# sandflow/ffmpeg-ht

Measured on AMD Instinct MI355X. Metric: Mpixels/s HTJ2K decode (4K lossless 5/3) at 1/2/4/8 GPU; IDWT HBM GB/s vs peak, higher is better.
Workload: dtype int32 (int16 storage); 1 GPU; configs[1]: 3840x2160 RGB 8-bit lossless 5/3 + RCT, 64x64 codeblocks, 5 levels, single tile, HT cleanup pass only; 128 frames per step per GPU as 2 concurrent jobs (HIP streams; the frame pipeline keeps that many in flight), device-resident input (codeblock bytes + descriptors) and output (rgb24); jobs=2, distinct_frames=4, block_errors=0

## Files before the change

ffmpeg-ht_amd/csrc/ht_kernels.hpp:

```cpp
#pragma once
#include <hip/hip_runtime.h>
#include <stdint.h>
#include "j2k_plan.h"

namespace htj2k {

struct HtLds {
    uint32_t off_ms, ms_words;
    uint32_t off_vlc, vlc_words;
    uint32_t off_suf, suf_bytes;
    uint32_t off_qinfo, max_qw;
    uint32_t off_E;
    uint32_t off_bm, bm_words;
    uint32_t total;
};

#define HT_ERR_INVALID 1
#define HT_REF_STRIDE 64
#define HT_MEL_SYMS  1344
#define HT_MEL_WORDS (HT_MEL_SYMS / 32 + 2)
#define HT_UVLC_ENTRIES (5 * 64)
#define HT_VSTAGE_PITCH 17
#define HT_VSTAGE_BYTES (64 * HT_VSTAGE_PITCH * 4)

// ... 269 lines not shown
        pv[jx] = pi * 8 < Pcup ? Dq[pi] : make_uint2(0u, 0u);
    }
#pragma unroll
    for (int jx = 0; jx < 4; jx++)
        if (512u * jx < Pcup) ht_unstuff_magsgn_step8(pv[jx], 64 * jx, Pcup, ms, lane, base, carry);
    for (uint32_t p0 = 256; p0 * 8 < Pcup; p0 += 64) {
        const uint32_t pi = p0 + lane;
        ht_unstuff_magsgn_step8(pi * 8 < Pcup ? Dq[pi] : make_uint2(0u, 0u), p0, Pcup, ms, lane, base, carry);
    }
    return base;
}

template <int TRANSFORM, bool REFINE, bool C16 = false>
__device__ __forceinline__ int ht_magsgn_rows_narrow(const ht_sym_t *__restrict__ qglob, const uint32_t *ms,
                                                     uint32_t *__restrict__ dst, int lane, int w, int h,
                                                     int stride, int pLSB, int maxbp, int M_b, float fscale, int i_step,
                                                     uint32_t last_wi, uint32_t *__restrict__ sink,
                                                     const uint64_t *__restrict__ rb, int z_blk)
{
    const int qw = (w + 1) >> 1, qh = (h + 1) >> 1;
    const int col = lane;
    const bool act = col < 2 * qw;
    const bool st_ok = col < w;
    const int q = col >> 1, sh = (col & 1) * 2;
    const int dshift = 31 - M_b;
    const uint32_t half = 1u << ((pLSB - 1) & 31);
    const bool direct53 = pLSB >= dshift && pLSB >= 1 && pLSB <= 30;
    const uint32_t keep53 = (uint32_t)(31 - pLSB) & 31u, up53 = (uint32_t)(pLSB - dshift) & 31u, hb53 = (half & 0x7FFFFFFFu) >> (dshift & 31);
    uint32_t ms_pos = 0, Eb = 0;
    int err = 0;
    const int qwp = (int)ht_qsym_pitch((uint32_t)w);
    const ht_sym_t *qp = qglob + q;
    uint32_t qi_next = act ? *qp : 0u;
    uint32_t *prow = dst + col;
    uint16_t *prow16 = (uint16_t *)dst + col;
    for (int row = 0; row < qh; row++) {
        const uint32_t qi = qi_next;
        qp += qwp;
        if (row + 1 < qh) qi_next = act ? *qp : 0u;
        const uint32_t rho = (qi | (qi >> 1)) & 0x55, uq = qi >> 8;
        const uint32_t f_t = (qi >> (2 * sh)) & 3, f_b = (qi >> (2 * sh + 2)) & 3;
        const uint32_t s_t = min(f_t, 1u), s_b = min(f_b, 1u);
        const uint32_t k_t = f_t >> 1, k_b = f_b >> 1;
        const uint32_t e_t = (f_t + 1) >> 2, e_b = (f_b + 1) >> 2;
        int kappa = 1;
        if (row > 0) {
            const uint32_t nbm = max(ht_dpp_left(Eb), ht_dpp_right(Eb));
            const uint32_t pm = max(Eb, ht_dpp_swap_pair(Eb));
            const int me = (int)max(pm, max(nbm, ht_dpp_swap_pair(nbm)));
            kappa = (rho & (rho - 1)) ? max(me - 1, 1) : 1;
        }
        const int U = kappa + (int)uq;
        if (act && U > maxbp) err = 1;
        const int m_t = __mul24((int)s_t, U) - (int)k_t, m_b = __mul24((int)s_b, U) - (int)k_b;
        const uint32_t nt = (uint32_t)max(m_t, 0), nb = (uint32_t)max(m_b, 0);
        const uint32_t incl = wave_incl_scan_u32(nt + nb, lane);
        const uint32_t pos = ms_pos + incl - nt - nb;
        ms_pos += wave_last(incl);
        const uint32_t wi = min(pos >> 5, last_wi), bs = pos & 31;
        const uint32_t w0 = ms[wi], w1 = ms[wi + 1], w2 = ms[wi + 2];
        uint32_t vt = __builtin_amdgcn_ubfe(__builtin_amdgcn_alignbit(w1, w0, bs), 0u, nt);
        const uint32_t sb = bs + nt;
        const bool hiw = sb >= 32;
        uint32_t vb = __builtin_amdgcn_ubfe(__builtin_amdgcn_alignbit(hiw ? w2 : w1, hiw ? w1 : w0, sb), 0u, nb);
        vt += e_t << nt;
        vb += e_b << nb;
        Eb = m_b != 0 ? (uint32_t)(32 - __clz((int)(vb | 1))) : 0u;
        uint32_t mu_t = 0, mu_b = 0;
        if (REFINE || TRANSFORM != J2K_DWT53 || !direct53) {
            mu_t = ((((vt >> 1) + 1) << pLSB) | half) | (vt << 31);
            mu_b = ((((vb >> 1) + 1) << pLSB) | half) | (vb << 31);
            mu_t = m_t != 0 ? mu_t : 0u;
            mu_b = m_b != 0 ? mu_b : 0u;
        }
        const bool two = 2 * row + 1 < h;
        if (REFINE) {
            const int qq = (pLSB - 1) & 31;
            const uint64_t *r = rb + (size_t)6 * row * HT_REF_STRIDE;
            const uint64_t Rt = r[0], Gt = r[HT_REF_STRIDE], Qt = r[2 * HT_REF_STRIDE];
            uint64_t Rb = 0, Gb = 0, Qb = 0;
            if (two) { Rb = r[3 * HT_REF_STRIDE]; Gb = r[4 * HT_REF_STRIDE]; Qb = r[5 * HT_REF_STRIDE]; }
            auto refine = [&](uint32_t v, uint32_t sig, uint64_t R, uint64_t G, uint64_t Q) -> uint32_t {
                const uint32_t nsig = (uint32_t)(R >> col) & 1u, sgn = (uint32_t)(G >> col) & 1u, mrb = (uint32_t)(Q >> col) & 1u;
                if (nsig) v |= (1u << qq) | (1u << ((qq - 1) & 31)) | (sgn << 31);
                if (z_blk > 2 && sig) { v &= (0xFFFFFFFEu | mrb) << qq; v |= 1u << ((qq - 1) & 31); }
                if (TRANSFORM == J2K_DWT_RAW) v &= ht_raw_mask(sig != 0, pLSB, z_blk);
                return v;
            };
            const uint32_t o_t = TRANSFORM == J2K_DWT_RAW ? ht_raw_index(refine(mu_t, s_t, Rt, Gt, Qt), M_b)
                                                          : ht_dequant(refine(mu_t, s_t, Rt, Gt, Qt), TRANSFORM, M_b, 0, fscale, i_step);
            const uint32_t o_b = TRANSFORM == J2K_DWT_RAW ? ht_raw_index(refine(mu_b, s_b, Rb, Gb, Qb), M_b)
                                                          : ht_dequant(refine(mu_b, s_b, Rb, Gb, Qb), TRANSFORM, M_b, 0, fscale, i_step);
            *(st_ok ? prow : sink) = o_t;
            *((st_ok && two) ? prow + stride : sink) = o_b;
        } else {
            uint32_t o_t, o_b;
            if (TRANSFORM == J2K_DWT53) {
                int r_t, r_b;
                if (direct53) {
                    const int sg_t = -(int)(vt & 1), sg_b = -(int)(vb & 1);
                    r_t = (int)((__builtin_amdgcn_ubfe((vt >> 1) + 1, 0u, keep53) << up53) | hb53);
                    r_b = (int)((__builtin_amdgcn_ubfe((vb >> 1) + 1, 0u, keep53) << up53) | hb53);
                    r_t = (r_t ^ sg_t) - sg_t;
                    r_b = (r_b ^ sg_b) - sg_b;
                    r_t = m_t != 0 ? r_t : 0;
                    r_b = m_b != 0 ? r_b : 0;
                } else {
                    const int sg_t = (int)mu_t >> 31, sg_b = (int)mu_b >> 31;
                    r_t = (int)((mu_t & 0x7FFFFFFFu) >> dshift); r_b = (int)((mu_b & 0x7FFFFFFFu) >> dshift);
                    r_t = (r_t ^ sg_t) - sg_t;
                    r_b = (r_b ^ sg_b) - sg_b;
                }
                if (i_step != 32768) {
                    const long long a = (long long)r_t * i_step, b2 = (long long)r_b * i_step;
                    r_t = (int)(a < 0 ? -((-a) >> 16) : (a >> 16));
                    r_b = (int)(b2 < 0 ? -((-b2) >> 16) : (b2 >> 16));
                }
                o_t = (uint32_t)r_t; o_b = (uint32_t)r_b;
            } else if (TRANSFORM == J2K_DWT97) {
                o_t = __float_as_uint((float)(mu_t & 0x7FFFFFFFu) * fscale) | (mu_t & 0x80000000u);
                o_b = __float_as_uint((float)(mu_b & 0x7FFFFFFFu) * fscale) | (mu_b & 0x80000000u);
            } else if (TRANSFORM == J2K_DWT_RAW) {
                o_t = ht_raw_index(mu_t & ht_raw_mask(true, pLSB, 1), M_b);
                o_b = ht_raw_index(mu_b & ht_raw_mask(true, pLSB, 1), M_b);
            } else {
                o_t = ht_dequant(mu_t, TRANSFORM, M_b, 0, fscale, i_step);
                o_b = ht_dequant(mu_b, TRANSFORM, M_b, 0, fscale, i_step);
            }
            if (C16) {
                *(st_ok ? prow16 : (uint16_t *)sink) = (uint16_t)o_t;
                *((st_ok && two) ? prow16 + stride : (uint16_t *)sink) = (uint16_t)o_b;
            } else {
                *(st_ok ? prow : sink) = o_t;
                *((st_ok && two) ? prow + stride : sink) = o_b;
            }
        }
        prow += 2 * stride;
        prow16 += 2 * stride;
    }
    return __any(err) ? HT_ERR_INVALID : 0;
}

__device__ __forceinline__ uint32_t half_incl_scan_u32(uint32_t v)
{
    int x = (int)v;
    x += __builtin_amdgcn_update_dpp(0, x, 0x111, 0xf, 0xf, false);
    x += __builtin_amdgcn_update_dpp(0, x, 0x112, 0xf, 0xf, false);
    x += __builtin_amdgcn_update_dpp(0, x, 0x114, 0xf, 0xf, false);
    x += __builtin_amdgcn_update_dpp(0, x, 0x118, 0xf, 0xf, false);
    x += __builtin_amdgcn_update_dpp(0, x, 0x142, 0xa, 0xf, false);
    return (uint32_t)x;
}

__global__ void __launch_bounds__(64)
k_ht_decode_pair(const J2kBlock *__restrict__ blocks, int nblocks, const uint8_t *__restrict__ bytes,
                 uint32_t *__restrict__ coef, int *__restrict__ status, uint32_t ms_words,
                 const ht_sym_t *__restrict__ qsym, const uint32_t *__restrict__ qoff, uint32_t *__restrict__ sink)
{
    extern __shared__ __align__(16) uint8_t smem[];
    uint32_t *ms_all = (uint32_t *)smem;
    const int lane = threadIdx.x, hf = lane >> 5, q = lane & 31;
    const uint32_t mspitch = ms_words + 4;
    bool ok_h[2] = { false, false };
    uint32_t lastwi_h[2] = { 0, 0 }, Pcup_h[2] = { 0, 0 };
    const uint32_t *Dw_h[2] = { nullptr, nullptr };
    uint2 pv[2][4];

    const int bi = min(2 * (int)blockIdx.x + hf, nblocks - 1);
    uint32_t sy[16];
    {
        const uint32_t wh = *(const uint32_t *)&blocks[bi].w;
        const int w_l = (int)(wh & 0xFFFFu), qw_l = (w_l + 1) >> 1;
        const uint32_t qwp_l = ht_qsym_pitch((uint32_t)w_l);
        const ht_sym_t *qp0 = qsym + qoff[bi] + (q < qw_l ? q : 0);
#pragma unroll
        for (int k = 0; k < 16; k++) {
            const uint32_t a = qp0[0], c = qp0[qwp_l];
            sy[k] = a | (c << 16);
            qp0 += 2 * qwp_l;
        }
        if (q >= qw_l) {
#pragma unroll
            for (int k = 0; k < 16; k++) sy[k] = 0;
        }
    }

#pragma unroll
    for (int hb = 0; hb < 2; hb++) {
#pragma unroll
        for (int jx = 0; jx < 4; jx++) pv[hb][jx] = make_uint2(0u, 0u);
        const int bidx = 2 * (int)blockIdx.x + hb;
        if (bidx >= nblocks) continue;
        const J2kBlock b = blocks[bidx];
        uint16_t *dst16 = (uint16_t *)coef + b.plane_off;
        if (b.npasses == 0) {
            ht_zero_window16(dst16, b.w, b.h, b.stride, lane);
            continue;
        }
        const int rem = b.npasses % 3, num_plhd = rem ? b.npasses - rem : b.npasses - 3;
        const int S_blk = (num_plhd / 3 + b.zbp) & 0xFF, maxbp = S_blk + 1;
        const uint32_t Lcup = b.lcup;
        const uint8_t *D = bytes + b.data_off;
        Dw_h[hb] = (const uint32_t *)D;
#pragma unroll
        for (int jx = 0; jx < 4; jx++) {
            const uint32_t pi = 64 * jx + lane;
            if (pi * 8 < Lcup) pv[hb][jx] = ((const uint2 *)Dw_h[hb])[pi];
        }
        int err = 0;
        uint32_t Scup = 0, Pcup = 0;
        if (Lcup < 2) err = HT_ERR_INVALID;
        if (!err) {
            Scup = (uint32_t)__builtin_amdgcn_readfirstlane((int)(((uint32_t)D[Lcup - 1] << 4) + (D[Lcup - 2] & 0x0F)));
            if (Scup < 2 || Scup > Lcup || Scup > 4079) err = HT_ERR_INVALID;
            Pcup = Lcup - Scup;
        }
        if (!err && maxbp >= 32) err = HT_ERR_INVALID;
        if (!err && (Pcup * 8 + 31) / 32 + 3 > ms_words) err = HT_ERR_INVALID;
        if (err) {
            ht_zero_window16(dst16, b.w, b.h, b.stride, lane);
            if (lane == 0) status[bidx] = err;
            continue;
        }
        ok_h[hb] = true;
        Pcup_h[hb] = Pcup;
    }
#pragma unroll
    for (int hb = 0; hb < 2; hb++) {
        if (!ok_h[hb]) continue;
        const uint32_t Pcup = Pcup_h[hb];
        uint32_t *ms = ms_all + hb * mspitch;
        const uint32_t nms = (Pcup * 8 + 31) / 32 + 2;
        ht_ms_clear(ms, nms + 2, lane);
        __syncthreads();
        uint32_t ms_total = 0, carry = 0;
#pragma unroll
        for (int jx = 0; jx < 4; jx++)
            if (512u * jx < Pcup) ht_unstuff_magsgn_step8(pv[hb][jx], 64 * jx, Pcup, ms, lane, ms_total, carry);
        for (uint32_t p0 = 256; p0 * 8 < Pcup; p0 += 64) {
            const uint32_t pi = p0 + lane;
            ht_unstuff_magsgn_step8(pi * 8 < Pcup ? ((const uint2 *)Dw_h[hb])[pi] : make_uint2(0u, 0u), p0, Pcup, ms, lane, ms_total, carry);
        }
        __syncthreads();
        ht_ms_ones_tail(ms, ms_total, nms + 1, lane);
        lastwi_h[hb] = nms - 2;
    }
    __syncthreads();
    if (!ok_h[0] && !ok_h[1]) return;

    const J2kBlock b = blocks[bi];
    const bool ok = hf ? ok_h[1] : ok_h[0];
    const int w = b.w, h = b.h, stride = b.stride, M_b = b.M_b;
    const int qw = (w + 1) >> 1, qh = ok ? (h + 1) >> 1 : 0;
    const int rem = b.npasses % 3, num_plhd = rem ? b.npasses - rem : b.npasses - 3;
    const int S_blk = (num_plhd / 3 + b.zbp) & 0xFF;
    const int pLSB = (30 - S_blk) & 0xFF, maxbp = S_blk + 1, dshift = 31 - M_b;
    const uint32_t halfbit = 1u << ((pLSB - 1) & 31);
    const uint32_t *ms = ms_all + hf * mspitch;
    const uint32_t last_wi = hf ? lastwi_h[1] : lastwi_h[0];
    const bool act = ok && q < qw;
    const int qwp = (int)ht_qsym_pitch((uint32_t)w);
    const ht_sym_t *qp = qsym + qoff[bi] + q;
    uint16_t *prow = (uint16_t *)coef + b.plane_off + 2 * q;
    const int rows = max(__builtin_amdgcn_readlane(qh, 0), __builtin_amdgcn_readlane(qh, 32));
    uint32_t qi_next = (act && qh > 0) ? *qp : 0u;
    uint32_t E1p = 0, E3p = 0, ms_pos = 0;
    int err = 0;
    const bool fast_blk = !ok || (pLSB >= dshift && pLSB >= 1 && pLSB <= 30 && maxbp <= 16);
    if (__ballot(!fast_blk) == 0) {
        const uint32_t up = (uint32_t)(pLSB - dshift) & 31u, hb = (halfbit & 0x7FFFFFFFu) >> (dshift & 31);
        const uint32_t LmHi = q == 0 ? 0u : 0xFFFF0000u, RmLo = q == 31 ? 0u : 0x0000FFFFu;
        const uint32_t mul2 = ((1u << up) & 0xFFFFu) * 0x00010001u, add2 = (((1u << up) | hb) & 0xFFFFu) * 0x00010001u;
        typedef unsigned short u16x2 __attribute__((ext_vector_type(2)));
        auto fast_rows = [&](auto simple_tag, auto pre_tag) {
        constexpr bool SIMPLE = decltype(simple_tag)::value, PRE = decltype(pre_tag)::value;
        uint16_t *pt = (SIMPLE && !act) ? (uint16_t *)sink : prow;
        const int st = (SIMPLE && !act) ? 0 : stride;
        uint32_t Zb = 0;
        uint32_t Umax = 0;
        const uint32_t minus2 = 0xFFFEFFFEu;
        auto quad_row = [&](int row, uint32_t sym, auto hi_tag) {
            constexpr bool HI = decltype(hi_tag)::value;
            const bool arow = SIMPLE ? act : (act && row < qh);
            const uint32_t pk = HI ? (sym >> 16) & 0xFFu : sym & 0xFFu, uq = HI ? sym >> 24 : (sym >> 8) & 0xFFu;
            const uint32_t pk2 = pk | (pk << 12);
            const uint32_t F = (pk2 | (pk2 << 6)) & 0x03030303u, Fh = F >> 1;
            const uint32_t R = (F | Fh) & 0x01010101u, K = Fh & 0x01010101u, X1 = F & Fh;
            uint32_t Z = (ht_dpp_left(Zb) & LmHi) | Zb;
            Z = (ht_dpp_right(Zb) & RmLo) | Z;
            const uint32_t Zf = ((Z >> 16) | Z | 1u) & 0xFFFFu;
            const int em2 = max(30 - (int)__builtin_clz(Zf), 0);
            const bool gamma = __builtin_amdgcn_sad_u8(R, 0u, 0u) > 1u;
            const uint32_t U = (gamma ? (uint32_t)em2 : 0u) + 1u + uq;
            if (SIMPLE) Umax = max(Umax, U);
            else if (arow && (int)U > maxbp) err = 1;
            uint32_t Rs = R << 8;
            asm("" : "+v"(Rs));
            const uint32_t Rm = Rs - R;
            const uint32_t U4 = __builtin_amdgcn_perm(U, U, 0x00000000u);
            const uint32_t N = (U4 - K) & Rm;
            const uint32_t tot = __builtin_amdgcn_sad_u8(N, 0u, 0u);
            const uint32_t incl = half_incl_scan_u32(tot);
            const uint32_t pos = ms_pos + incl - tot;
            ms_pos += (uint32_t)__builtin_amdgcn_ds_swizzle((int)incl, 31 << 5);
            const uint32_t wi = min(pos >> 5, last_wi + 1);
            const uint32_t w0 = ms[wi], w1 = ms[wi + 1], w2 = ms[wi + 2];
            uint32_t lo = __builtin_amdgcn_alignbit(w1, w0, pos), hi = __builtin_amdgcn_alignbit(w2, w1, pos);
            const uint32_t N1 = N >> 8, N2 = N >> 16, N3 = N >> 24;
            const uint32_t v0 = __builtin_amdgcn_ubfe(lo, 0u, N);
            lo = __builtin_amdgcn_alignbit(hi, lo, N); hi = __builtin_amdgcn_alignbit(0u, hi, N);
            const uint32_t v1 = __builtin_amdgcn_ubfe(lo, 0u, N1);
            lo = __builtin_amdgcn_alignbit(hi, lo, N1); hi = __builtin_amdgcn_alignbit(0u, hi, N1);
            const uint32_t v2 = __builtin_amdgcn_ubfe(lo, 0u, N2);
            lo = __builtin_amdgcn_alignbit(hi, lo, N2);
            const uint32_t v3 = __builtin_amdgcn_ubfe(lo, 0u, N3);
            uint32_t xt, xb, sgB, X1b;
            asm("v_pk_lshrrev_b16 %0, 8, %1 op_sel_hi:[0,1]" : "=v"(sgB) : "v"(R));
            asm("v_pk_lshrrev_b16 %0, 8, %1 op_sel_hi:[0,1]" : "=v"(X1b) : "v"(X1));
            asm("v_pk_lshlrev_b16 %0, %1, %2" : "=v"(xt) : "v"(N), "v"(X1 & 0x00010001u));
            asm("v_pk_lshlrev_b16 %0, %1, %2" : "=v"(xb) : "v"(N1), "v"(X1b));
            const uint32_t Pt = __builtin_amdgcn_perm(v2, v0, 0x05040100u) | xt, Pb = __builtin_amdgcn_perm(v3, v1, 0x05040100u) | xb;
            const uint32_t sgT = R & 0x00010001u;
            Zb = Pb | sgB;
            auto samples = [&](uint32_t P, uint32_t sig) -> uint32_t {
                const u16x2 r = (__builtin_bit_cast(u16x2, P) >> (u16x2){ 1, 1 }) * __builtin_bit_cast(u16x2, mul2) + __builtin_bit_cast(u16x2, add2);
                uint32_t m;
                asm("v_pk_mad_i16 %0, %1, %2, %3" : "=v"(m) : "v"(P & 0x00010001u), "v"(minus2), "v"(sig));
                return __builtin_bit_cast(uint32_t, (u16x2)(r * __builtin_bit_cast(u16x2, m)));
            };
            const uint32_t top = samples(Pt, sgT), bot = samples(Pb, sgB);
            if (SIMPLE) {
                *(uint32_t *)pt = top;
                *(uint32_t *)(pt + st) = bot;
            } else {
                const bool two = 2 * row + 1 < h;
                *(arow ? (uint32_t *)pt : sink) = top;
                *((arow && two) ? (uint32_t *)(pt + st) : sink) = bot;
            }
            pt += 2 * st;
        };
        if (PRE) {
            for (int k = 0; 2 * k < rows; k++) {
                uint32_t s2 = sy[k];
                if (!SIMPLE) {
                    s2 = (act && 2 * k < qh) ? s2 : 0u;
                    s2 = (2 * k + 1 < qh) ? s2 : s2 & 0xFFFFu;
                }
                quad_row(2 * k, s2, std::false_type{});
                if (2 * k + 1 < rows) quad_row(2 * k + 1, s2, std::true_type{});
            }
        } else {
            for (int row = 0; row < rows; row++) {
                const uint32_t qi = qi_next;
                qp += qwp;
                qi_next = (act && row + 1 < (SIMPLE ? rows : qh)) ? *qp : 0u;
                quad_row(row, qi, std::false_type{});
            }
        }
        if (SIMPLE && act && (int)Umax > maxbp) err = 1;
        };
        const int qh0 = __builtin_amdgcn_readlane(qh, 0), qh1 = __builtin_amdgcn_readlane(qh, 32);
        const bool simple = qh0 == qh1 && __ballot(ok && (h & 1)) == 0;
        if (rows <= 32) {
            if (simple) fast_rows(std::true_type{}, std::true_type{}); else fast_rows(std::false_type{}, std::true_type{});
        } else {
            if (simple) fast_rows(std::true_type{}, std::false_type{}); else fast_rows(std::false_type{}, std::false_type{});
        }
    } else
    for (int row = 0; row < rows; row++) {
        const bool arow = act && row < qh;
        const uint32_t qi = qi_next;
        qp += qwp;
        qi_next = (act && row + 1 < qh) ? *qp : 0u;
        const uint32_t qx = ht_sym_unpack(qi);
        const uint32_t rho = qx & 0xF, ek = (qx >> 4) & 0xF, e1 = (qx >> 8) & 0xF, uq = (qx >> 16) & 0xFF;
        int kappa = 1;
        if (row > 0) {
            uint32_t l = ht_dpp_left(E3p), r = ht_dpp_right(E1p);
            l = q == 0 ? 0u : l;
            r = q == 31 ? 0u : r;
            const int me = (int)max(max(E1p, E3p), max(l, r));
            kappa = (rho & (rho - 1)) ? max(me - 1, 1) : 1;
        }
        const int U = kappa + (int)uq;
        if (arow && U > maxbp) err = 1;
        const int m0 = __mul24((int)(rho & 1), U) - (int)(ek & 1), m1 = __mul24((int)((rho >> 1) & 1), U) - (int)((ek >> 1) & 1);
        const int m2 = __mul24((int)((rho >> 2) & 1), U) - (int)((ek >> 2) & 1), m3 = __mul24((int)((rho >> 3) & 1), U) - (int)((ek >> 3) & 1);
        const uint32_t n0 = (uint32_t)max(m0, 0), n1 = (uint32_t)max(m1, 0), n2 = (uint32_t)max(m2, 0), n3 = (uint32_t)max(m3, 0);
        const uint32_t tot = n0 + n1 + n2 + n3;
        const uint32_t incl = half_incl_scan_u32(tot);
        const uint32_t pos = ms_pos + incl - tot;
        ms_pos += (uint32_t)__builtin_amdgcn_ds_swizzle((int)incl, 31 << 5);
        auto cut = [&](uint32_t p, uint32_t n) -> uint32_t {
            const uint32_t i = min(p >> 5, last_wi + 2);
            return __builtin_amdgcn_ubfe(__builtin_amdgcn_alignbit(ms[i + 1], ms[i], p), 0u, n);
        };
        const uint32_t p1 = pos + n0, p2 = p1 + n1, p3 = p2 + n2;
        uint32_t v0 = cut(pos, n0), v1 = cut(p1, n1), v2 = cut(p2, n2), v3 = cut(p3, n3);
// ... 277 lines not shown
                dB = (d0 >> 2) | ((d1 >> 2) << 2);
            } else {
                Qt = (dB & 1u) | ((dB >> 1) & 2u);
                Qb = ((dB >> 1) & 1u) | ((dB >> 2) & 2u);
            }
            if (refined && row < qh) {
                const uint32_t *r = rg + (size_t)(2 * row) * 2 * MW;
                if (MW == 1) {
                    Rt = r[0] >> (2 * q); Gt = r[1] >> (2 * q);
                    if (2 * row + 1 < h) { Rb = r[2] >> (2 * q); Gb = r[3] >> (2 * q); }
                } else {
                    Rt = (uint32_t)((((uint64_t)r[1] << 32) | r[0]) >> (2 * q)); Gt = (uint32_t)((((uint64_t)r[3] << 32) | r[2]) >> (2 * q));
                    if (2 * row + 1 < h) { Rb = (uint32_t)((((uint64_t)r[5] << 32) | r[4]) >> (2 * q)); Gb = (uint32_t)((((uint64_t)r[7] << 32) | r[6]) >> (2 * q)); }
                }
            }
        }
        auto sample = [&](uint32_t v, int sm, uint32_t nsig, uint32_t sgn, uint32_t mrb) -> uint32_t {
            uint32_t mu = (((((v >> 1) + 1u) << pLSB) | halfbit) | (v << 31)) & (uint32_t)sm;
            if (REFINE) {
                mu |= ((sgn << 31) | ref_new) & (uint32_t)-(int)(nsig & 1u);
                const uint32_t keep = ((mrb & 1u) << qq_) | ref_keep | ~(uint32_t)sm;
                mu = (mu & keep) | (ref_half & (uint32_t)sm);
                if (TRANSFORM == J2K_DWT_RAW) return ht_raw_index(mu & ht_raw_mask(sm != 0, pLSB, z_blk), M_b);
                if (TRANSFORM == J2K_DWT97) return __float_as_uint((float)(mu & 0x7FFFFFFFu) * fscale) | (mu & 0x80000000u);
                return ht_dequant(mu, TRANSFORM, M_b, 0, fscale, i_step);
            }
            if (TRANSFORM == J2K_DWT_RAW) return ht_raw_index(mu & ht_raw_mask(true, pLSB, 1), M_b);
            if (TRANSFORM == J2K_DWT53) {
                const int sg = (int)mu >> 31;
                int r = (int)((mu & 0x7FFFFFFFu) >> dshift);
                r = (r ^ sg) - sg;
                if (i_step != 32768) {
                    const long long a = (long long)r * i_step;
                    r = (int)(a < 0 ? -((-a) >> 16) : (a >> 16));
                }
                return (uint32_t)r;
            } else if (TRANSFORM == J2K_DWT97) {
                return __float_as_uint((float)(mu & 0x7FFFFFFFu) * fscale) | (mu & 0x80000000u);
            } else {
                return ht_dequant(mu, TRANSFORM, M_b, 0, fscale, i_step);
            }
        };
        const uint32_t o0 = sample(v0, s0m, Rt, Gt & 1, Qt);
        const uint32_t o1 = sample(v1, s1m, Rb, Gb & 1, Qb);
        const uint32_t o2 = sample(v2, s2m, Rt >> 1, (Gt >> 1) & 1, Qt >> 1);
        const uint32_t o3 = sample(v3, s3m, Rb >> 1, (Gb >> 1) & 1, Qb >> 1);
        const bool two = 2 * row + 1 < h;
        if (pairs) {
            u32x2 t, bt;
            t.x = o0; t.y = o2; bt.x = o1; bt.y = o3;
            *(u32x2_a4 *)(arow ? prow : sink) = t;
            *(u32x2_a4 *)((arow && two) ? prow + stride : sink) = bt;
        } else {
            *(arow ? prow : sink) = o0;
            *((arow && c2) ? prow + 1 : sink) = o2;
            *((arow && two) ? prow + stride : sink) = o1;
            *((arow && two && c2) ? prow + stride + 1 : sink) = o3;
        }
        prow += 2 * stride;
    };
    if (pre) {
        for (int k = 0; 2 * k < rows; k++) {
            uint32_t s2 = sy[k];
            s2 = (act && 2 * k < qh) ? s2 : 0u;
            s2 = (2 * k + 1 < qh) ? s2 : s2 & 0xFFFFu;
            quad_row(2 * k, s2 & 0xFFFFu, s2 >> 16);
            if (2 * k + 1 < rows) quad_row(2 * k + 1, s2 >> 16, 0u);
        }
    } else {
        for (int row = 0; row < rows; row++) {
            const uint32_t qi = qi_next;
            qp += qwp;
            qi_next = (act && row + 1 < qh) ? *qp : 0u;
            quad_row(row, qi, qi_next);
        }
    }
#pragma unroll
    for (int hb = 0; hb < NB; hb++) {
        if (__ballot(err && seg == hb) == 0) continue;
        const int bidx = NB * (int)blockIdx.x + hb;
        const J2kBlock bb = blocks[bidx];
        __syncthreads();
        ht_zero_window(coef + bb.plane_off, bb.w, bb.h, bb.stride, lane);
        if (lane == 0) status[bidx] = HT_ERR_INVALID;
    }
}

#define HT_DECODE_KERNEL k_ht_decode
#define HT_DECODE_RAW 0
#include "ht_decode_block.hpp"
#undef HT_DECODE_KERNEL
#undef HT_DECODE_RAW
#define HT_DECODE_KERNEL k_ht_decode_raw
#define HT_DECODE_RAW 1
#include "ht_decode_block.hpp"
#undef HT_DECODE_KERNEL
#undef HT_DECODE_RAW


__device__ __forceinline__ void ht_unstuff_backward_step8(uint2 dq, uint32_t k0, uint32_t n, uint32_t first_or,
                                                          uint32_t *out, int lane, uint32_t &base, uint32_t &carry)
{
    const uint32_t k = k0 + 8 * lane;
    uint32_t lo = __builtin_bswap32(dq.y), hi = __builtin_bswap32(dq.x);
    if (k == 0) lo |= first_or;
    int nv = 8;
    if (k0 + 512 > n) {
        nv = min(max((int)n - (int)k, 0), 8);
        const int nl = min(nv, 4), nh = nv - nl;
        lo = nl == 4 ? lo : (nl ? lo & (0xFFFFFFFFu >> (32 - 8 * nl)) : 0u);
        hi = nh == 4 ? hi : (nh ? hi & (0xFFFFFFFFu >> (32 - 8 * nh)) : 0u);
    }
    const uint32_t ll = lo & 0x7F7F7F7Fu, lh = hi & 0x7F7F7F7Fu;
    const uint32_t Al = (ll + 0x70707070u) & lo & 0x80808080u, Ah = (lh + 0x70707070u) & hi & 0x80808080u;
    const uint32_t Bl = (ll + 0x01010101u) & 0x80808080u, Bh = (lh + 0x01010101u) & 0x80808080u;
    uint32_t prevA = ht_dpp_left(Ah >> 24);
    if (lane == 0) prevA = carry;
    carry = (uint32_t)__builtin_amdgcn_readlane((int)(Ah >> 24), 63);
    uint32_t fl = Bl & ((Al << 8) | prevA), fh = Bh & __builtin_amdgcn_alignbyte(Ah, Al, 3);
    if (nv < 8) {
        const int nl = min(nv, 4), nh = nv - nl;
        fl = nl == 4 ? fl : (nl ? fl & (0xFFFFFFFFu >> (32 - 8 * nl)) : 0u);
        fh = nh == 4 ? fh : (nh ? fh & (0xFFFFFFFFu >> (32 - 8 * nh)) : 0u);
    }
    ht_squeeze_place<false>(lo, hi, fl, fh, nv, out, lane, base);
}

__device__ __forceinline__ uint32_t ht_unstuff_backward(const uint8_t *__restrict__ top, uint32_t n, uint32_t first_or,
                                                        uint32_t *out, int lane)
{
    uint32_t base = 0, carry = 0x80;
    for (uint32_t k0 = 0; k0 < n; k0 += 512) {
        const uint32_t k = k0 + 8 * lane;
        uint2 dq = make_uint2(0u, 0u);
        if (k < n) __builtin_memcpy(&dq, top - k - 7, 8);
        ht_unstuff_backward_step8(dq, k0, n, first_or, out, lane, base, carry);
    }
    return base;
}

__device__ __forceinline__ uint32_t ht_unstuff_forward7(const uint8_t *__restrict__ src, uint32_t n, uint32_t *out, int lane)
{
    uint32_t base = 0, carry = 0;
    for (uint32_t p0 = 0; p0 * 8 < n; p0 += 64) {
        const uint32_t i = (p0 + lane) * 8;
        uint2 dq = make_uint2(0u, 0u);
        if (i < n) __builtin_memcpy(&dq, src + i, 8);
        ht_unstuff_fwd_step8<false>(dq, p0, n, out, lane, base, carry);
    }
    return base;
}


template <int LPB>
__device__ __forceinline__ uint32_t grp_incl_scan_u32(uint32_t v)
{
    int x = (int)v;
    x += __builtin_amdgcn_update_dpp(0, x, 0x111, 0xf, 0xf, false);
    x += __builtin_amdgcn_update_dpp(0, x, 0x112, 0xf, 0xf, false);
    x += __builtin_amdgcn_update_dpp(0, x, 0x114, 0xf, 0xf, false);
    x += __builtin_amdgcn_update_dpp(0, x, 0x118, 0xf, 0xf, false);
    if (LPB >= 32) x += __builtin_amdgcn_update_dpp(0, x, 0x142, 0xa, 0xf, false);
    if (LPB >= 64) x += __builtin_amdgcn_update_dpp(0, x, 0x143, 0xc, 0xf, false);
    return (uint32_t)x;
}
template <int LPB>
__device__ __forceinline__ uint32_t grp_last(uint32_t v, int lane)
{
    return (uint32_t)__builtin_amdgcn_ds_bpermute((lane | (LPB - 1)) << 2, (int)v);
}
template <bool OR_SEM, int LPB>
__device__ __forceinline__ void ht_squeeze_place_g(uint32_t lo, uint32_t hi, uint32_t fl, uint32_t fh, int nv,
                                                   uint32_t *out, int lane, uint32_t &base)
{
    const uint32_t tot = 8u * (uint32_t)nv - (uint32_t)__builtin_popcount(fl) - (uint32_t)__builtin_popcount(fh);
    while (__ballot(fh != 0) != 0) {
        if (fh) {
            const uint32_t k = 31u - (uint32_t)__builtin_clz(fh), bit = 1u << k, m = bit - 1u;
            uint32_t nh = (hi & m) | ((hi >> 1) & ~m);
            if (OR_SEM) nh |= hi & bit;
            hi = nh;
            fh &= m;
        }
    }
    while (__ballot(fl != 0) != 0) {
        if (fl) {
            const uint32_t k = 31u - (uint32_t)__builtin_clz(fl), bit = 1u << k, m = bit - 1u;
            uint32_t nl = (lo & m) | (__builtin_amdgcn_alignbit(hi, lo, 1) & ~m);
            if (OR_SEM) nl |= lo & bit;
            lo = nl;
            hi >>= 1;
            fl &= m;
        }
    }
    const uint32_t incl = grp_incl_scan_u32<LPB>(tot);
    const uint32_t off = base + incl - tot;
    if (nv > 0) {
        const uint32_t sh = off & 31;
        const uint64_t t = (uint64_t)lo << sh, u = (uint64_t)hi << sh;
        uint32_t *o = out + (off >> 5);
        atomicOr(o, (uint32_t)t);
        atomicOr(o + 1, (uint32_t)(t >> 32) | (uint32_t)u);
        if (sh + tot + (OR_SEM ? 1u : 0u) > 64) atomicOr(o + 2, (uint32_t)(u >> 32));
    }
    base += grp_last<LPB>(incl, lane);
}
__device__ __forceinline__ uint32_t ht_first_bytes(uint32_t v, int n) { return n >= 4 ? v : (n > 0 ? v & (0xFFFFFFFFu >> (32 - 8 * n)) : 0u); }
template <int LPB>
__device__ __forceinline__ void ht_unstuff_backward_step8_g(uint2 dq, uint32_t k0, uint32_t n, uint32_t first_or,
                                                            uint32_t *out, int lane, uint32_t &base, uint32_t &carry)
{
    const int gl = lane & (LPB - 1);
    const uint32_t k = k0 + 8 * gl;
    const int nv = min(max((int)n - (int)k, 0), 8);
    uint32_t lo = __builtin_bswap32(dq.y), hi = __builtin_bswap32(dq.x);
    if (k == 0) lo |= first_or;
    lo = ht_first_bytes(lo, nv); hi = ht_first_bytes(hi, nv - 4);
    const uint32_t ll = lo & 0x7F7F7F7Fu, lh = hi & 0x7F7F7F7Fu;
    const uint32_t Al = (ll + 0x70707070u) & lo & 0x80808080u, Ah = (lh + 0x70707070u) & hi & 0x80808080u;
    const uint32_t Bl = (ll + 0x01010101u) & 0x80808080u, Bh = (lh + 0x01010101u) & 0x80808080u;
    uint32_t prevA = ht_dpp_left(Ah >> 24);
    if (gl == 0) prevA = carry;
    carry = grp_last<LPB>(Ah >> 24, lane);
    const uint32_t fl = ht_first_bytes(Bl & ((Al << 8) | prevA), nv), fh = ht_first_bytes(Bh & __builtin_amdgcn_alignbyte(Ah, Al, 3), nv - 4);
    ht_squeeze_place_g<false, LPB>(lo, hi, fl, fh, nv, out, lane, base);
}
template <int LPB>
__device__ __forceinline__ void ht_unstuff_fwd7_step8_g(uint2 dq, uint32_t p0, uint32_t n, uint32_t *out, int lane,
                                                        uint32_t &base, uint32_t &carry)
{
    const int gl = lane & (LPB - 1);
    const int nv = min(max((int)n - (int)(p0 + 8 * gl), 0), 8);
    const uint32_t lo = ht_first_bytes(dq.x, nv), hi = ht_first_bytes(dq.y, nv - 4);
    uint32_t prev = ht_dpp_left(hi >> 24);
    if (gl == 0) prev = carry;
    carry = grp_last<LPB>(hi >> 24, lane);
    const uint32_t Pl = (lo << 8) | prev, Ph = __builtin_amdgcn_alignbyte(hi, lo, 3);
    const uint32_t fl = ht_first_bytes(((Pl & 0x7F7F7F7Fu) + 0x01010101u) & Pl & 0x80808080u, nv);
    const uint32_t fh = ht_first_bytes(((Ph & 0x7F7F7F7Fu) + 0x01010101u) & Ph & 0x80808080u, nv - 4);
    ht_squeeze_place_g<false, LPB>(lo, hi, fl, fh, nv, out, lane, base);
}

template <int LPB>
__global__ void __launch_bounds__(64)
k_ht_unstuff_g(const J2kBlock *__restrict__ blocks, int nblocks, const uint8_t *__restrict__ bytes,
               uint32_t *__restrict__ vlc_u, uint32_t *__restrict__ mel_u, uint32_t lds_words)
{
    extern __shared__ __align__(16) uint32_t sw[];
    constexpr int G = 64 / LPB;
    const int lane = threadIdx.x, gl = lane & (LPB - 1);
    const int bi = (int)blockIdx.x * G + lane / LPB;
    J2kBlock b;
    memset(&b, 0, sizeof(b));
    if (bi < nblocks) b = blocks[bi];
    const uint8_t *D = bytes + b.data_off;
    const uint32_t Lcup = b.lcup;
    bool ok = bi < nblocks && b.npasses != 0 && Lcup >= 2;
    uint2 pv[2];
#pragma unroll
    for (int j = 0; j < 2; j++) {
        const long long o = (long long)b.data_off + Lcup - 9 - (8 * LPB * j + 8 * gl);
        pv[j] = make_uint2(0u, 0u);
        if (ok && o >= 0) __builtin_memcpy(&pv[j], bytes + o, 8);
    }
    uint32_t Scup = 0;
    if (ok) Scup = ((uint32_t)D[Lcup - 1] << 4) + (D[Lcup - 2] & 0x0F);
    ok = ok && !(Scup < 2 || Scup > Lcup || Scup > 4079);
    const uint32_t nsw = ht_nsw(Scup);
    ok = ok && 2 * nsw <= lds_words;
    uint32_t *vlO = vlc_u + (b.data_off >> 2), *meO = mel_u + (b.data_off >> 2);
    uint32_t *sv = sw + (size_t)(lane / LPB) * lds_words;

    if (ok) for (uint32_t i = gl; i < nsw; i += LPB) sv[i] = 0;
    __syncthreads();
    {
        const uint8_t *top = D + Lcup - 2;
        const uint32_t n = ok ? Scup - 1 : 0u;
        uint32_t base = 0, carry = 0x80;
#pragma unroll
        for (int j = 0; j < 2; j++)
            if (__ballot((uint32_t)(8 * LPB * j) < n) != 0) ht_unstuff_backward_step8_g<LPB>(pv[j], 8 * LPB * j, n, 0x0F, sv, lane, base, carry);
        for (uint32_t k0 = 16 * LPB; __ballot(k0 < n) != 0; k0 += 8 * LPB) {
            const uint32_t k = k0 + 8 * gl;
            uint2 dq = make_uint2(0u, 0u);
            if (k < n) __builtin_memcpy(&dq, top - k - 7, 8);
            ht_unstuff_backward_step8_g<LPB>(dq, k0, n, 0x0F, sv, lane, base, carry);
        }
    }
    __syncthreads();
    if (ok) for (uint32_t i = gl; i < nsw; i += LPB) vlO[i] = sv[i];

    const int rem = b.npasses % 3, plhd = rem ? b.npasses - rem : b.npasses - 3;
    const uint32_t Lref = b.lref, nsp = ht_nsp(Lref);
    const bool ref = ok && b.npasses - plhd > 1 && Lref > 0 && 2 * nsp <= lds_words;
    if (__ballot(ref) == 0) return;
    uint32_t *ss = sv, *sr = sv + nsp;
    __syncthreads();
    if (ref) for (uint32_t i = gl; i < 2 * nsp; i += LPB) sv[i] = 0;
    __syncthreads();
    {
        const uint32_t n = ref ? Lref : 0u;
        uint32_t base = 0, carry = 0;
        for (uint32_t p0 = 0; __ballot(p0 < n) != 0; p0 += 8 * LPB) {
            const uint32_t i = p0 + 8 * gl;
            uint2 dq = make_uint2(0u, 0u);
            if (i < n) __builtin_memcpy(&dq, D + Lcup + i, 8);
            ht_unstuff_fwd7_step8_g<LPB>(dq, p0, n, ss, lane, base, carry);
        }
        base = 0; carry = 0x80;
        const uint8_t *top = D + Lcup + Lref - 1;
        for (uint32_t k0 = 0; __ballot(k0 < n) != 0; k0 += 8 * LPB) {
            const uint32_t k = k0 + 8 * gl;
            uint2 dq = make_uint2(0u, 0u);
            if (k < n) __builtin_memcpy(&dq, top - k - 7, 8);
            ht_unstuff_backward_step8_g<LPB>(dq, k0, n, 0, sr, lane, base, carry);
        }
    }
    __syncthreads();
    if (ref) for (uint32_t i = gl; i < nsp; i += LPB) {
        vlO[nsw + i] = ss[i];
        meO[nsw + i] = sr[i];
    }
}

__global__ void __launch_bounds__(64)
k_ht_unstuff(const J2kBlock *__restrict__ blocks, int nblocks, const uint8_t *__restrict__ bytes,
             uint32_t *__restrict__ vlc_u, uint32_t *__restrict__ mel_u, uint32_t lds_words)
{
    extern __shared__ __align__(16) uint32_t sw[];
    const int lane = threadIdx.x;
    if ((int)blockIdx.x >= nblocks) return;
    const J2kBlock b = blocks[blockIdx.x];
    if (b.npasses == 0 || b.lcup < 2) return;
    const uint8_t *D = bytes + b.data_off;
    const uint32_t Lcup = b.lcup;
    uint2 pv[2];
#pragma unroll
    for (int j = 0; j < 2; j++) {
        const long long o = (long long)b.data_off + Lcup - 9 - (512 * j + 8 * lane);
        pv[j] = make_uint2(0u, 0u);
        if (o >= 0) __builtin_memcpy(&pv[j], bytes + o, 8);
    }
    const uint32_t Scup = (uint32_t)__builtin_amdgcn_readfirstlane((int)(((uint32_t)D[Lcup - 1] << 4) + (D[Lcup - 2] & 0x0F)));
    if (Scup < 2 || Scup > Lcup || Scup > 4079) return;
    const uint32_t nsw = ht_nsw(Scup);
    if (2 * nsw > lds_words) return;
    uint32_t *vlO = vlc_u + (b.data_off >> 2), *meO = mel_u + (b.data_off >> 2);
    uint32_t *sv = sw;

    for (uint32_t i = lane; i < nsw; i += 64) sw[i] = 0;
    __syncthreads();

    {
        const uint8_t *top = D + Lcup - 2;
        const uint32_t n = Scup - 1;
        uint32_t base = 0, carry = 0x80;
#pragma unroll
        for (int j = 0; j < 2; j++)
            if (512u * j < n) ht_unstuff_backward_step8(pv[j], 512 * j, n, 0x0F, sv, lane, base, carry);
        for (uint32_t k0 = 1024; k0 < n; k0 += 512) {
// ... 772 lines not shown
```

Measured before the change: 174,000 Mpixel/s.

## Unstuff MagSgn for both codeblocks concurrently using half-wave 16-byte groups

The MagSgn unstuffing in the paired decode kernel used to run the whole 64-lane wave over each codeblock in turn, with 8 bytes per lane. Now each 32-lane half-wave processes its own codeblock at the same time, with 16 bytes per lane. A new squeeze/place routine handles four words per lane and only loops on lanes that hold more than one stuffing bit. This removes one serial pass and one barrier, and halves the preloaded register footprint. In exchange, per-lane ALU work rises, the handling of multiple stuff bits becomes more complex, and there are more atomicOr writes per lane.

```diff
diff --git a/ffmpeg-ht_amd/csrc/ht_kernels.hpp b/ffmpeg-ht_amd/csrc/ht_kernels.hpp
--- a/ffmpeg-ht_amd/csrc/ht_kernels.hpp
+++ b/ffmpeg-ht_amd/csrc/ht_kernels.hpp
@@ -445,6 +445,104 @@
     return (uint32_t)x;
 }
 
+template <int LPB>
+__device__ __forceinline__ uint32_t grp_incl_scan_u32(uint32_t v)
+{
+    int x = (int)v;
+    x += __builtin_amdgcn_update_dpp(0, x, 0x111, 0xf, 0xf, false);
+    x += __builtin_amdgcn_update_dpp(0, x, 0x112, 0xf, 0xf, false);
+    x += __builtin_amdgcn_update_dpp(0, x, 0x114, 0xf, 0xf, false);
+    x += __builtin_amdgcn_update_dpp(0, x, 0x118, 0xf, 0xf, false);
+    if (LPB >= 32) x += __builtin_amdgcn_update_dpp(0, x, 0x142, 0xa, 0xf, false);
+    if (LPB >= 64) x += __builtin_amdgcn_update_dpp(0, x, 0x143, 0xc, 0xf, false);
+    return (uint32_t)x;
+}
+template <int LPB>
+__device__ __forceinline__ uint32_t grp_last(uint32_t v, int lane)
+{
+    return (uint32_t)__builtin_amdgcn_ds_bpermute((lane | (LPB - 1)) << 2, (int)v);
+}
+__device__ __forceinline__ uint32_t ht_first_bytes(uint32_t v, int n) { return n >= 4 ? v : (n > 0 ? v & (0xFFFFFFFFu >> (32 - 8 * n)) : 0u); }
+
+template <bool OR_SEM>
+__device__ __forceinline__ void ht_drop_bit16(uint32_t (&w)[4], uint32_t e0, uint32_t e1, uint32_t e2, uint32_t e3)
+{
+    unsigned c;
+    const uint32_t m0 = __builtin_subc(e0, 1u, 0u, &c), m1 = __builtin_subc(e1, 0u, c, &c);
+    const uint32_t m2 = __builtin_subc(e2, 0u, c, &c), m3 = __builtin_subc(e3, 0u, c, &c);
+    const uint32_t s0 = __builtin_amdgcn_alignbit(w[1], w[0], 1), s1 = __builtin_amdgcn_alignbit(w[2], w[1], 1);
+    const uint32_t s2 = __builtin_amdgcn_alignbit(w[3], w[2], 1), s3 = w[3] >> 1;
+    uint32_t n0 = (w[0] & m0) | (s0 & ~m0), n1 = (w[1] & m1) | (s1 & ~m1);
+    uint32_t n2 = (w[2] & m2) | (s2 & ~m2), n3 = (w[3] & m3) | (s3 & ~m3);
+    if (OR_SEM) {
+        asm("" : "+v"(n0), "+v"(n1), "+v"(n2), "+v"(n3));
+        n0 |= w[0] & e0; n1 |= w[1] & e1; n2 |= w[2] & e2; n3 |= w[3] & e3;
+    }
+    w[0] = n0; w[1] = n1; w[2] = n2; w[3] = n3;
+}
+__device__ __forceinline__ uint32_t ht_top_bit(uint32_t f) { return f ? 0x80000000u >> __builtin_clz(f) : 0u; }
+
+template <bool OR_SEM, int LPB>
+__device__ __forceinline__ void ht_squeeze_place16_g(uint32_t (&w)[4], uint32_t f0, uint32_t f1, uint32_t f2, uint32_t f3, int nv,
+                                                     uint32_t *out, int lane, uint32_t &base)
+{
+    uint32_t cnt = (uint32_t)__builtin_popcount(f0) + (uint32_t)__builtin_popcount(f1) + (uint32_t)__builtin_popcount(f2) +
+                   (uint32_t)__builtin_popcount(f3);
+    const uint32_t tot = 8u * (uint32_t)nv - cnt;
+    if (__builtin_expect(__ballot(cnt > 1) != 0, 0)) {
+        do {
+            if (cnt > 1) {
+                const uint32_t e3 = ht_top_bit(f3), e2 = f3 ? 0u : ht_top_bit(f2), e1 = (f3 | f2) ? 0u : ht_top_bit(f1);
+                const uint32_t e0 = (f3 | f2 | f1) ? 0u : ht_top_bit(f0);
+                ht_drop_bit16<OR_SEM>(w, e0, e1, e2, e3);
+                f0 &= ~e0; f1 &= ~e1; f2 &= ~e2; f3 &= ~e3;
+                cnt--;
+            }
+        } while (__ballot(cnt > 1) != 0);
+    }
+    ht_drop_bit16<OR_SEM>(w, f0, f1, f2, f3);
+    const uint32_t incl = grp_incl_scan_u32<LPB>(tot);
+    const uint32_t off = base + incl - tot;
+    if (nv > 0) {
+        const uint32_t sh = off & 31, end = sh + tot + (OR_SEM ? 1u : 0u);
+        const uint64_t t0 = ((uint64_t)w[1] << 32 | w[0]) << sh, t1 = ((uint64_t)w[2] << 32 | w[1]) << sh;
+        const uint64_t t2 = ((uint64_t)w[3] << 32 | w[2]) << sh, t3 = (uint64_t)w[3] << sh;
+        uint32_t *o = out + (off >> 5);
+        atomicOr(o, (uint32_t)t0);
+        atomicOr(o + 1, (uint32_t)(t0 >> 32));
+        if (end > 64) atomicOr(o + 2, (uint32_t)(t1 >> 32));
+        if (end > 96) atomicOr(o + 3, (uint32_t)(t2 >> 32));
+        if (end > 128) atomicOr(o + 4, (uint32_t)(t3 >> 32));
+    }
+    base += grp_last<LPB>(incl, lane);
+}
+
+template <bool OR_SEM, int LPB>
+__device__ __forceinline__ void ht_unstuff_fwd_step16_g(uint4 dq, uint32_t p0, uint32_t n, uint32_t *out, int lane,
+                                                        uint32_t &base, uint32_t &carry)
+{
+    const int gl = lane & (LPB - 1);
+    const int nv = min(max((int)n - (int)(p0 + 16 * gl), 0), 16);
+    uint32_t w[4] = { dq.x, dq.y, dq.z, dq.w };
+    uint32_t V[4] = { 0x80808080u, 0x80808080u, 0x80808080u, 0x80808080u };
+    if (__ballot(nv < 16) != 0) {
+#pragma unroll
+        for (int i = 0; i < 4; i++) {
+            const uint32_t keep = ht_first_bytes(0xFFFFFFFFu, nv - 4 * i);
+            w[i] &= keep;
+            V[i] &= keep;
+        }
+    }
+    uint32_t prev = ht_dpp_left(w[3] >> 24);
+    if (gl == 0) prev = carry;
+    carry = grp_last<LPB>(w[3] >> 24, lane);
+    const uint32_t P0 = (w[0] << 8) | prev, P1 = __builtin_amdgcn_alignbyte(w[1], w[0], 3);
+    const uint32_t P2 = __builtin_amdgcn_alignbyte(w[2], w[1], 3), P3 = __builtin_amdgcn_alignbyte(w[3], w[2], 3);
+    const uint32_t f0 = ((P0 & 0x7F7F7F7Fu) + 0x01010101u) & P0 & V[0], f1 = ((P1 & 0x7F7F7F7Fu) + 0x01010101u) & P1 & V[1];
+    const uint32_t f2 = ((P2 & 0x7F7F7F7Fu) + 0x01010101u) & P2 & V[2], f3 = ((P3 & 0x7F7F7F7Fu) + 0x01010101u) & P3 & V[3];
+    ht_squeeze_place16_g<OR_SEM, LPB>(w, f0, f1, f2, f3, nv, out, lane, base);
+}
+
 __global__ void __launch_bounds__(64)
 k_ht_decode_pair(const J2kBlock *__restrict__ blocks, int nblocks, const uint8_t *__restrict__ bytes,
                  uint32_t *__restrict__ coef, int *__restrict__ status, uint32_t ms_words,
@@ -456,8 +554,9 @@
     const uint32_t mspitch = ms_words + 4;
     bool ok_h[2] = { false, false };
     uint32_t lastwi_h[2] = { 0, 0 }, Pcup_h[2] = { 0, 0 };
-    const uint32_t *Dw_h[2] = { nullptr, nullptr };
-    uint2 pv[2][4];
+    uint4 pv[4];
+#pragma unroll
+    for (int jx = 0; jx < 4; jx++) pv[jx] = make_uint4(0u, 0u, 0u, 0u);
 
     const int bi = min(2 * (int)blockIdx.x + hf, nblocks - 1);
     uint32_t sy[16];
@@ -480,8 +579,6 @@
 
 #pragma unroll
     for (int hb = 0; hb < 2; hb++) {
-#pragma unroll
-        for (int jx = 0; jx < 4; jx++) pv[hb][jx] = make_uint2(0u, 0u);
         const int bidx = 2 * (int)blockIdx.x + hb;
         if (bidx >= nblocks) continue;
         const J2kBlock b = blocks[bidx];
@@ -494,11 +591,10 @@
         const int S_blk = (num_plhd / 3 + b.zbp) & 0xFF, maxbp = S_blk + 1;
         const uint32_t Lcup = b.lcup;
         const uint8_t *D = bytes + b.data_off;
-        Dw_h[hb] = (const uint32_t *)D;
 #pragma unroll
         for (int jx = 0; jx < 4; jx++) {
-            const uint32_t pi = 64 * jx + lane;
-            if (pi * 8 < Lcup) pv[hb][jx] = ((const uint2 *)Dw_h[hb])[pi];
+            const uint32_t pi = (32 * jx + q) * 16;
+            if (hf == hb && pi < Lcup) __builtin_memcpy(&pv[jx], D + pi, 16);
         }
         int err = 0;
         uint32_t Scup = 0, Pcup = 0;
@@ -519,24 +615,31 @@
         Pcup_h[hb] = Pcup;
     }
 #pragma unroll
-    for (int hb = 0; hb < 2; hb++) {
-        if (!ok_h[hb]) continue;
-        const uint32_t Pcup = Pcup_h[hb];
-        uint32_t *ms = ms_all + hb * mspitch;
-        const uint32_t nms = (Pcup * 8 + 31) / 32 + 2;
-        ht_ms_clear(ms, nms + 2, lane);
+    for (int hb = 0; hb < 2; hb++)
+        if (ok_h[hb]) ht_ms_clear(ms_all + hb * mspitch, (Pcup_h[hb] * 8 + 31) / 32 + 4, lane);
+    __syncthreads();
+    {
+        const uint32_t Pl = hf ? Pcup_h[1] : Pcup_h[0];
+        const uint8_t *Dl = bytes + blocks[bi].data_off;
+        uint32_t *msl = ms_all + hf * mspitch;
+        uint32_t ms_total = 0, carry = 0;
+#pragma unroll
+        for (int jx = 0; jx < 4; jx++)
+            if (__ballot(512u * jx < Pl) != 0) ht_unstuff_fwd_step16_g<true, 32>(pv[jx], 512u * jx, Pl, msl, lane, ms_total, carry);
+        for (uint32_t p0 = 2048; __ballot(p0 < Pl) != 0; p0 += 512) {
+            const uint32_t pi = p0 + 16 * q;
+            uint4 dq = make_uint4(0u, 0u, 0u, 0u);
+            if (pi < Pl) __builtin_memcpy(&dq, Dl + pi, 16);
+            ht_unstuff_fwd_step16_g<true, 32>(dq, p0, Pl, msl, lane, ms_total, carry);
+        }
         __syncthreads();
-        uint32_t ms_total = 0, carry = 0;
-#pragma unroll
-        for (int jx = 0; jx < 4; jx++)
-            if (512u * jx < Pcup) ht_unstuff_magsgn_step8(pv[hb][jx], 64 * jx, Pcup, ms, lane, ms_total, carry);
-        for (uint32_t p0 = 256; p0 * 8 < Pcup; p0 += 64) {
-            const uint32_t pi = p0 + lane;
-            ht_unstuff_magsgn_step8(pi * 8 < Pcup ? ((const uint2 *)Dw_h[hb])[pi] : make_uint2(0u, 0u), p0, Pcup, ms, lane, ms_total, carry);
-        }
-        __syncthreads();
-        ht_ms_ones_tail(ms, ms_total, nms + 1, lane);
-        lastwi_h[hb] = nms - 2;
+#pragma unroll
+        for (int hb = 0; hb < 2; hb++) {
+            if (!ok_h[hb]) continue;
+            const uint32_t nms = (Pcup_h[hb] * 8 + 31) / 32 + 2;
+            ht_ms_ones_tail(ms_all + hb * mspitch, (uint32_t)__builtin_amdgcn_readlane((int)ms_total, 32 * hb), nms + 1, lane);
+            lastwi_h[hb] = nms - 2;
+        }
     }
     __syncthreads();
     if (!ok_h[0] && !ok_h[1]) return;
@@ -1120,23 +1223,6 @@
 }
 
 
-template <int LPB>
-__device__ __forceinline__ uint32_t grp_incl_scan_u32(uint32_t v)
-{
-    int x = (int)v;
-    x += __builtin_amdgcn_update_dpp(0, x, 0x111, 0xf, 0xf, false);
-    x += __builtin_amdgcn_update_dpp(0, x, 0x112, 0xf, 0xf, false);
-    x += __builtin_amdgcn_update_dpp(0, x, 0x114, 0xf, 0xf, false);
-    x += __builtin_amdgcn_update_dpp(0, x, 0x118, 0xf, 0xf, false);
-    if (LPB >= 32) x += __builtin_amdgcn_update_dpp(0, x, 0x142, 0xa, 0xf, false);
-    if (LPB >= 64) x += __builtin_amdgcn_update_dpp(0, x, 0x143, 0xc, 0xf, false);
-    return (uint32_t)x;
-}
-template <int LPB>
-__device__ __forceinline__ uint32_t grp_last(uint32_t v, int lane)
-{
-    return (uint32_t)__builtin_amdgcn_ds_bpermute((lane | (LPB - 1)) << 2, (int)v);
-}
 template <bool OR_SEM, int LPB>
 __device__ __forceinline__ void ht_squeeze_place_g(uint32_t lo, uint32_t hi, uint32_t fl, uint32_t fh, int nv,
                                                    uint32_t *out, int lane, uint32_t &base)
@@ -1173,7 +1259,6 @@
     }
     base += grp_last<LPB>(incl, lane);
 }
-__device__ __forceinline__ uint32_t ht_first_bytes(uint32_t v, int n) { return n >= 4 ? v : (n > 0 ? v & (0xFFFFFFFFu >> (32 - 8 * n)) : 0u); }
 template <int LPB>
 __device__ __forceinline__ void ht_unstuff_backward_step8_g(uint2 dq, uint32_t k0, uint32_t n, uint32_t first_or,
                                                             uint32_t *out, int lane, uint32_t &base, uint32_t &carry)
```

Measured after the change: 173,400 Mpixel/s (median of 3 runs). About the same (-0.3%).
